# ishine/tts-max

Hardware: AMD Instinct MI355X
Metric: audio-codes/sec + RTF@24kHz, TTS-1 bs=1/32, at 1/2/4/8 MI355X (higher is better)
Workload: dtype bf16; 1 GPU; tts1 bf16 bs=1/GPU: prompt 202 tokens (150 codes), 500 greedy codes, codec codec-24k on 650 codes; model=TTS-1 (Llama-3.2-1B dims, V=193856, tied) + xcodec2-style codec codec-24k, global_batch=1, seq_len=702, parallelism=dp1

## Files before the change

### include/tts_mi355x_ops.h

```cpp
#ifndef TTS_MI355X_OPS_H
#define TTS_MI355X_OPS_H

#include <stdint.h>
#include "tts_mi355x.h"

#ifdef __cplusplus
extern "C" {
#endif

tts_status tts_synth_fill(void* dst, int32_t dtype, int64_t n, uint64_t seed, float scale,
                          void* stream);

tts_status tts_op_retile(const void* w, void* w_tiled, int32_t N, int32_t K, int32_t epi, void* stream);

tts_status tts_op_wgemm(const void* x, int32_t M, int32_t K, int32_t ldx, const void* w_tiled,
                        int32_t N, const void* normw, float eps, void* out, int32_t ldo,
                        void* resid, int32_t epi, void* stream);

tts_status tts_op_pgemm(const void* x, int32_t M, int32_t K, const void* w_tiled, int32_t N, void* out,
                        int32_t ldo, void* resid, int32_t epi, void* stream);

tts_status tts_op_head_pick(const void* x, int32_t M, int32_t K, const void* normw, float eps, const void* w_tiled,
                            int32_t N, const uint32_t* seen, int32_t seen_stride, float penalty,
                            const uint16_t* counts, float freq_penalty, const int32_t* eos_mask,
// ... 3 lines not shown
tts_status tts_op_sample(const float* logits, int32_t B, int32_t V, float temperature, int32_t top_k,
                         float top_p, uint64_t seed, int32_t step, const float* part_max, int32_t nparts,
                         float* probs, int32_t* tokens, void* stream);

tts_status tts_op_sample_list(const float* scores, const int32_t* ids, const int32_t* counts, int32_t B,
                              int32_t cap, int32_t V, float temperature, int32_t top_k, float top_p, uint64_t seed,
                              int32_t step, float* probs, int32_t* tokens, void* stream);

tts_status tts_op_sample_rows(const float* scores, const int32_t* ids, const int32_t* counts, int32_t B, int32_t cap,
                              int32_t V, const float* temperature, const int32_t* top_k, const float* top_p,
                              const int32_t* sample, const uint64_t* row_seed, int32_t step, const float* part_max,
                              const int32_t* part_idx, int32_t nparts, float* probs, int32_t* tokens, void* stream);

tts_status tts_debug_step_plan(const tts_lm_config* cfg, int32_t rows, int32_t num_cu, char* out, int32_t cap);
tts_status tts_debug_wgemm_plan(int32_t M, int32_t N, int32_t K, int32_t epi, int32_t num_cu, int32_t* out);
tts_status tts_debug_step_plan_sampled(const tts_lm_config* cfg, int32_t rows, int32_t num_cu, int32_t top_k,
                                       char* out, int32_t cap);

tts_status tts_debug_step_plan_rows(const tts_lm_config* cfg, int32_t rows, int32_t num_cu, int32_t max_top_k,
                                    char* out, int32_t cap);

tts_status tts_op_rmsnorm(const void* x, const void* w, float eps, void* y, int32_t M, int32_t K,
                          void* stream);

tts_status tts_op_attn_prefill(const void* qkv, int32_t ld_qkv, const int32_t* seq_slot, const int32_t* seq_pos0,
                               const int32_t* seq_len, int32_t n_seq, int32_t n_slots, void* kcache,
                               void* vtcache, int32_t max_seq, const void* rope_cos, const void* rope_sin,
                               int32_t H, int32_t KVH, int32_t D, float scale, void* q_rot, void* out,
                               void* stream);

// ... 15 lines not shown
```

### tts-max_amd/csrc/capi.cpp

```cpp
#include <stdlib.h>
#include <string.h>

#include <algorithm>
#include <memory>
#include <string>

#include "../../include/tts_mi355x.h"
#include "../../include/tts_mi355x_ops.h"
#include "codec_kernels.h"
#include "engine.h"

namespace tts {

static thread_local std::string g_last_error;

template <class F>
static tts_status guarded(F&& f) {
  try {
    f();
    return TTS_OK;
  } catch (const Error& e) {
    g_last_error = e.what();
    return e.code;
  } catch (const std::exception& e) {
// ... 242 lines not shown
}

tts_status tts_debug_wgemm_plan(int32_t M, int32_t N, int32_t K, int32_t epi, int32_t num_cu, int32_t* out) {
  return guarded([&] {
    TTS_REQUIRE(out && num_cu > 0, "null argument");
    TTS_REQUIRE(epi >= EPI_STORE && epi <= EPI_LOGITS_ROWS && wgemm_supported(M, N, K, epi), "unsupported GEMM shape");
    const WgemmPlan p = plan_wgemm(M, N, K, epi, num_cu);
    out[0] = (N / 16) / p.sp.ng;
    out[1] = p.sp.ur();
    out[2] = p.grid;
    out[3] = p.sp.kc;
    out[4] = p.csplit;
    out[5] = p.sliced ? 1 : 0;
    out[6] = p.a_lds ? 1 : 0;
    out[7] = p.cfg;
  });
}

tts_status tts_debug_step_plan_sampled(const tts_lm_config* cfg, int32_t rows, int32_t num_cu, int32_t top_k,
                                       char* out, int32_t cap) {
  return guarded([&] {
    TTS_REQUIRE(cfg && out && cap > 0, "null argument");
    TTS_REQUIRE(top_k >= 1 && top_k <= SAMPLE_MAX_TOP_K, "top_k in [1, 1024]");
    const std::string p = lm_step_plan(*cfg, rows, num_cu, top_k);
    TTS_REQUIRE((int64_t)p.size() < cap, "output buffer too small");
    memcpy(out, p.c_str(), p.size() + 1);
  });
}

tts_status tts_debug_step_plan_rows(const tts_lm_config* cfg, int32_t rows, int32_t num_cu, int32_t max_top_k,
// ... 415 lines not shown
```

### tts-max_amd/csrc/lm_debug.cpp

```cpp
#include "lm_step.h"

namespace tts {

#ifdef TTS_STAMPS
static unsigned long long* g_stamps = nullptr;
constexpr int kStampSlots = 1 << 16;
unsigned long long* stamp_buf() {
  if (!g_stamps) {
    HIP_CHECK(hipMalloc((void**)&g_stamps, kStampSlots * 8));
    HIP_CHECK(hipMemset(g_stamps, 0, kStampSlots * 8));
  }
  return g_stamps;
}
extern "C" int tts_debug_stamps(unsigned long long* host, int n) {
  if (!g_stamps || n > kStampSlots) return 1;
  if (hipDeviceSynchronize() != hipSuccess) return 1;
  if (hipMemcpy(host, g_stamps, (size_t)n * 8, hipMemcpyDeviceToHost) != hipSuccess) return 1;
  return hipMemset(g_stamps, 0, kStampSlots * 8) == hipSuccess ? 0 : 1;
}
#else
unsigned long long* stamp_buf() { return nullptr; }
#endif

void lm_bench_kernel(Engine* e, int which, int rows, int ctx, int iters, float* avg_ms,
                     double* bytes) {
  TTS_REQUIRE(e->lm.loaded, "tts_lm_load has not been called");
  TTS_REQUIRE(rows >= 1 && rows <= e->w.cap_batch, "rows out of range");
  TTS_REQUIRE(ctx >= 1 && ctx <= e->lm.cfg.max_seq_len, "ctx out of range");
  TTS_REQUIRE(which >= 0 && which <= 11 && iters >= 1, "bad kernel selector");
  hipStream_t s = e->stream;
  Ctx X(e, s);
  const tts_lm_config& c = X.c;
  const int HID = c.hidden_size, HD = c.num_heads * c.head_dim, FF = c.intermediate_size;
  const int V = c.vocab_size, QKV = X.QKV(), hgrid = X.M.head_grid;
  TTS_REQUIRE(which < 6 || which > 7 || X.fused_attn_ok(rows, true), "fused QKV+attention does not apply to this shape");
  TTS_REQUIRE(which != 10 || (hgrid && head_screen_topk_supported(rows, HID, V, 50, hgrid)),
              "the screened sampling head does not apply to this shape (or is off)");
  TTS_REQUIRE(which < 8 || which > 9 || (hgrid && rows <= 32 && head_screen_supported(rows, HID, V)),
              "the screened lm_head does not apply to this shape (or is off)");
  TTS_REQUIRE(which != 7 || (rows == 1 ? X.fused_oproj_ok() : X.fused_oproj_rows_ok(rows)),
              "fused o_proj does not apply to this shape (or is off)");
  std::vector<int> tok(rows), pos(rows, ctx - 1);
  for (int r = 0; r < rows; ++r) tok[r] = (r * 7919 + 11) % V;
  HIP_CHECK(hipMemcpyAsync(e->w.row_idx.p, tok.data(), rows * 4, hipMemcpyHostToDevice, s));
// ... 70 lines not shown
          X.pending_norm = nullptr;
          X.screened_sample(e->w.x.as<bf16_t>(), rows, st, sampled);
          b = (double)V * HID + 16.0 * V + act_rw * HID + rows * (V / 8.0);
        } else {
          X.pending_norm = nullptr;
          X.lm_head_pick(e->w.x.as<bf16_t>(), rows, sx, EPI_LOGITS, true);
          SampleArgs sa = X.sample_args(st, sampled, false, X.head_parts(rows, EPI_LOGITS, true));
          sa.out_part_val = nullptr; sa.out_part_idx = nullptr;
          sa.tokens = e->w.row_idx.as<int>();
          launch_sample(sa, rows, s);
          b = 2.0 * V * HID + act_rw * HID + 2.0 * HID + rows * (V / 8.0) + 2.0 * rows * V * 4.0;
        }
        launch_bump_epoch(st.epoch, s);
        break;
      }
    }
  };
  launch();
  HIP_CHECK(hipGetLastError());
  HIP_CHECK(hipEventRecord(e->ev[2], s));
  for (int i = 0; i < iters; ++i) launch();
  HIP_CHECK(hipEventRecord(e->ev[3], s));
  HIP_CHECK(hipEventSynchronize(e->ev[3]));
  float ms = 0.f;
  HIP_CHECK(hipEventElapsedTime(&ms, e->ev[2], e->ev[3]));
  *avg_ms = ms / iters;
  *bytes = b;
  read_device_flags(e, s);
}

// ... 87 lines not shown
```

### tts-max_amd/csrc/lm_gemm.hip

```cpp
#include <algorithm>
#include <cstdio>
#include <stdexcept>

#include "env.h"
#include "lm_gemm_kernel.h"

namespace tts {

std::vector<std::string>*& dry_launches() {
  static thread_local std::vector<std::string>* rec = nullptr;
  return rec;
}

__global__ void retile_kernel(const bf16_t* __restrict__ w, bf16_t* __restrict__ t, int N,
                              int K, int nt_mult, int nt_off, StreamPlan p, int units) {
  const int KT = K / 32;
  const long long nchunks = (long long)(N / 16) * KT * 64;
  const int ur = p.ur();
  for (long long c = blockIdx.x * (long long)blockDim.x + threadIdx.x; c < nchunks;
       c += (long long)gridDim.x * blockDim.x) {
    const int lane = (int)(c & 63);
    const long long tile = c >> 6;
    const int kt = (int)(tile % KT);
    const int nt = (int)(tile / KT);
// ... 127 lines not shown
  return M >= 1 && M <= 64 && N > 0 && K > 0 && (N % (16 * NG)) == 0 && (K % 256) == 0 &&
         (unsigned long long)N * (unsigned long long)K * 2ull <= kWgemmMaxBytes;
}

void launch_wgemm(const WgemmArgs& a_in, const WgemmPlan& p_in, int epi, bool norm, hipStream_t s) {
  WgemmArgs a = a_in;
  WgemmPlan p = p_in;
  if (p.csplit == 2 && a.fattn_wgs) {
    p.csplit = 1;
    p.grid = p.sp.grid;
  }
  a.ur = p.sp.ur();
  a.kc = p.sp.kc;
  a.sliced = p.sliced ? 1 : 0;
  a.csplit = p.csplit;
  if (a.csplit == 2 && epi != EPI_STORE && epi != EPI_RESID)
    throw std::runtime_error("wgemm: column split only for plain store / residual launches");
  static const int diag = env_int("TTS_WGEMM_DIAG", 0);
  a.diag = diag;
  if (p.sliced) {
    if (norm || (epi != EPI_STORE && epi != EPI_RESID) || (a.part_out == nullptr && !dry_launches()))
      throw std::runtime_error("K-sliced wgemm: store/residual epilogues with a partial workspace only");
    const int Kfull = a.K;
    a.K = Kfull / p.sp.kc;
    launch_wgemm_store(a, p, false, s);
    if (epi == EPI_RESID && a.next_norm && !a.norm_out && !dry_launches())
      throw std::runtime_error("K-sliced wgemm: next_norm without norm_out");
    if (epi == EPI_RESID && a.next_norm)
      launch_splitk_combine_norm(a.part_out, p.sp.kc, a.M, a.N, a.ldo, a.resid, a.ldo, a.next_norm, a.eps,
                                 a.norm_out, a.ldo, s);
// ... 17 lines not shown
```

### tts-max_amd/csrc/lm_gemm_kernel.h

```cpp
#pragma once
#include <algorithm>
#include <cstdio>
#include <stdexcept>
#include <type_traits>

#include "hip_common.h"
#include "lm_kernels.h"
#include "lm_attn_core.h"
#include "lm_logit_epilogue.h"

namespace tts {

constexpr int wgemm_ea(int waves) { return waves >= 16 ? 1 : (waves >= 8 ? 2 : 4); }
__host__ __device__ inline int wgemm_red_floats(int waves, int ksplit, int ng, int mt, int M, int Kl) {
  const int upw = waves / ksplit;
  int r = upw * (ksplit - 1) * ng * mt * 4 * 64;
  r = r > upw * mt * 16 * 2 ? r : upw * mt * 16 * 2;
  const int segs = (M * (Kl / 8) + 63) / 64;
  r = r > segs ? r : segs;
  r = r > Kl / 2 ? r : Kl / 2;
  return r + 64;
}

constexpr int wgemm_fattn_d(int ku) { return ku == 2 ? 64 : 128; }
// ... 215 lines not shown
      for (int j = 0; j < HB; ++j)
        if (p0 + j < KSPLIT) pv[j] = *(const f32x4_t*)(red + ((size_t)(p0 + j - 1) * 64 + lane) * 4);
#pragma unroll
      for (int j = 0; j < HB; ++j)
        if (p0 + j < KSPLIT) acc += pv[j];
    }
#pragma unroll
    for (int r = 0; r < 4; ++r) {
      const int m = 4 * (lane >> 4) + r;
      if (m < M) a.fo_resid[(size_t)m * hid + u * 16 + (lane & 15)] = f2bf(bf2f(rr[r]) + rbf(acc[r]));
    }
  }
  TTS_STAMP(stp, 3);
}


constexpr int A_GLOBAL = 0, A_LDS = 1;

template <int WAVES, int KU, int MT_MAX, int NG, int KSPLIT, int ASRC, bool NORM, int EPI, int R,
          bool EARLY, int KSW = KSPLIT, bool FROWS = false>
__global__ __launch_bounds__(WAVES * 64) void wgemm_kernel(WgemmArgs a) {
  extern __shared__ __attribute__((aligned(16))) char smem[];
  constexpr int NT = WAVES * 64;
  constexpr bool LOGITS = EPI == EPI_LOGITS || EPI == EPI_LOGITS_ROWS;
  constexpr bool FATT = EPI == EPI_STORE && ASRC == A_LDS && WAVES == DEC_NW && KSW == KSPLIT && MT_MAX == 1 &&
                        ((EARLY && !FROWS && wgemm_fattn_d(KU) == 64) || (!EARLY && FROWS));
#ifdef TTS_STAMPS
  const unsigned long long t_first = __builtin_amdgcn_s_memrealtime();
#endif
  asm volatile("" ::"s"(a.x), "s"(a.w), "s"(a.normw), "s"(a.resid), "s"(a.stamps), "s"(a.M), "s"(a.K), "s"(a.ldx),
               "s"(a.N), "s"(a.ldo), "s"(a.ur));
  asm volatile("" ::"s"(a.fattn_wgs), "s"(a.fo_units), "s"(a.csplit), "s"(a.sliced), "s"(a.diag), "s"(a.KT), "s"(a.Sc),
               "s"(a.S), "s"(a.units), "s"(a.nproj), "s"(a.ur_div.mul), "s"(a.ur_div.shift), "s"(a.kch_div.mul),
               "s"(a.kch_div.shift), "s"(a.sc_div.mul), "s"(a.sc_div.shift));
  const int nproj = FROWS ? (int)gridDim.x - a.fattn_wgs - (a.fattn_wgs ? a.fo_units : 0) : a.nproj;
  if constexpr (FATT) {
    const int cb = (int)blockIdx.x - nproj;
    if (FROWS ? a.fattn_wgs != 0 : cb >= 0) {
      if (cb >= 0 && cb < a.fattn_wgs) {
        fattn_consumer<NT, wgemm_fattn_d(KU)>(a, smem, cb);
        return;
      }
      if (cb >= a.fattn_wgs) {
        const int lane = threadIdx.x & 63;
        const int wave = __builtin_amdgcn_readfirstlane(threadIdx.x >> 6);
        const size_t xs_bytes = (((size_t)a.M * (a.K + 8) * 2 + 15) & ~(size_t)15);
        if constexpr (FROWS) {
          fused_oproj_rows<KU, KSPLIT, R>(a, (bf16_t*)smem, (float*)(smem + xs_bytes), wave, lane, cb - a.fattn_wgs);
        } else {
          const uint32_t tag = ((uint32_t)a.fa.row_pos[0] << 6) | (uint32_t)a.fattn_layer;
          fused_oproj<KU, KSPLIT, R>(a, (bf16_t*)smem, (float*)(smem + xs_bytes), wave, lane, tag, cb - a.fattn_wgs);
        }
        return;
      }
    }
  }
// ... 23 lines not shown
  const int st_off = SL > 1 ? 0 : by * Sc;
  const int kt_base = by * (a.K >> 5);
  const bf16_t* xg = a.x + (uint32_t)(by * a.K);
  const int ldxs = a.K + 8;
  const int ustride = nproj * UPW;

  bf16_t* xs = (bf16_t*)smem;
  const size_t xs_bytes = (ASRC != A_GLOBAL) ? (((size_t)M * ldxs * 2 + 15) & ~(size_t)15) : 0;
  float* red = (float*)(smem + xs_bytes);

  const int ur = a.ur;
  auto stile = [&](int uu, int st) -> long long {
    uu = min(uu, units - 1) >> cs2;
    const int r = (int)fastdiv((uint32_t)uu, a.ur_div), ui = uu - r * ur;
    const int nr = min(ur, bunits - r * ur);
    return (long long)r * ur * KT * NG + (((long long)(st + st_off) * nr + ui) * KSPLIT + kpart) * NG * KU;
  };
  const int S = a.S;

  const int tid = threadIdx.x;
  const int kch = a.K >> 3;
  constexpr bool FTAGS = FATT && !EARLY;
  int ftag_pos = 0;
  if constexpr (FTAGS) {
    if (a.fattn_wgs) ftag_pos = a.fa.row_pos[min(lane & 15, M - 1)];
  }
  constexpr int EA = wgemm_ea(WAVES);
  const int achunks = M * kch;
  const int a_nj = (achunks + NT - 1) / NT;
  constexpr bool early_a = EARLY && ASRC == A_LDS;
  u32x4_t xe[EA], ne[EA];
// ... 495 lines not shown
      throw std::runtime_error("wgemm: fused one-row attention: head dim 64 only");
    if (a.fo_units && a.M > 1) {
      const int HD = a.fa.H * a.fa.D;
      const int S = (HD / 32) / (KSPLIT * KU);
      if (!(a.fo_w && a.fo_resid && a.fo_units <= a.fo_ur && S == R && KSPLIT == WAVES && HD == a.K && a.fo_kc >= 1 &&
            (HD / 32) % (a.fo_kc * KSPLIT * KU) == 0 && R * KU % 4 == 0 && R * KU >= 4))
        throw std::runtime_error("wgemm: fused multi-row o_proj shape mismatch");
    } else if (a.fo_units) {
      const int S = (a.fa.H * a.fa.D / 32) / (KSPLIT * KU);
      if (!(a.fo_w && a.fo_resid && a.fo_units <= a.fo_ur && S == R && a.fa.H * a.fa.D == KSPLIT * 128 &&
            KSPLIT == WAVES && (size_t)a.M * (a.K + 8) * 2 >= (size_t)KSPLIT * 256))
        throw std::runtime_error("wgemm: fused o_proj shape mismatch");
    }
    lds = std::max(lds, a.fa.D == 64 ? fattn_lds_bytes<64>() : fattn_lds_bytes<128>());
    grid += a.fattn_wgs + a.fo_units;
  }
  if (lds > 160 * 1024) throw std::runtime_error("wgemm: LDS request above 160 KiB");
  if ((unsigned long long)a.N * (unsigned long long)(a.sliced ? (size_t)a.K * a.kc : (size_t)a.K) * 2ull > kWgemmMaxBytes)
    throw std::runtime_error("wgemm: tiled weight matrix above the 32-bit buffer range");
  if (ASRC == A_LDS && !EARLY && a.K % 512 != 0)
    throw std::runtime_error("wgemm: the LDS-DMA prologue needs K a multiple of 512 (plan_wgemm: A_GLOBAL)");
  wgemm_derive(a, KU, NG, KSPLIT, KSPLIT, nproj, ASRC != A_GLOBAL);
  const dim3 g(grid, a.sliced ? a.kc : 1);
  if (!a.x) throw std::runtime_error("wgemm: launch without an A operand");
  if (g.y != 1 && !a.sliced) throw std::runtime_error("wgemm: grid.y > 1 on an unsliced launch");
  if (frows) {
    if constexpr (EPI == EPI_STORE && ASRC == A_LDS && WAVES == DEC_NW)
      hipLaunchKernelGGL((wgemm_kernel<WAVES, KU, 1, NG, KSPLIT, ASRC, NORM, EPI, R, false, KSPLIT, true>), g,
                         dim3(WAVES * 64), lds, s, a);
  } else if (mt == 1)
// ... 13 lines not shown
  if (a.M <= 16 && !(a.fattn_wgs && a.M > 1)) {
    const int kch = a.K / 8, NT = WAVES * 64;
    if (ASRC == A_LDS) early = (kch % 64 == 0) && (a.M * kch + NT - 1) / NT <= wgemm_ea(WAVES);
  }
  if constexpr (ASRC == A_GLOBAL) launch_one_e<WAVES, KU, NG, KSPLIT, ASRC, NORM, EPI, R, false>(a, grid, s);
  else if (early) launch_one_e<WAVES, KU, NG, KSPLIT, ASRC, NORM, EPI, R, true>(a, grid, s);
  else launch_one_e<WAVES, KU, NG, KSPLIT, ASRC, NORM, EPI, R, false>(a, grid, s);
}

template <int C, int NG, int ASRC, bool NORM, int EPI>
static void launch_shape(const WgemmArgs& a, int grid, hipStream_t s) {
  constexpr Shape3 h = kShapes[C];
  const int S = (a.K / 32) / (h.ksplit * h.ku);
  const bool agr_r1 = ASRC == A_GLOBAL && (h.ku >= 4 || (a.M > 16 && h.ku > 2));
  if constexpr (NG == 2 && ASRC == A_LDS && h.ku == 2 && h.waves == 8) {
    if (a.M >= 4 && a.M <= 32 && S % 4 == 0) {
      launch_one<h.waves, h.ku, NG, h.ksplit, ASRC, NORM, EPI, 4>(a, grid, s);
      return;
    }
  }
  if (h.r >= 2 && S % 2 == 0 && !agr_r1) launch_one<h.waves, h.ku, NG, h.ksplit, ASRC, NORM, EPI, 2>(a, grid, s);
  else launch_one<h.waves, h.ku, NG, h.ksplit, ASRC, NORM, EPI, 1>(a, grid, s);
}

template <int NG, int ASRC, bool NORM, int EPI>
static void launch_cfg(const WgemmArgs& a, int cfg, int grid, hipStream_t s) {
  if constexpr (NG == 2) {
    switch (cfg) {
      case 4: launch_shape<4, NG, ASRC, NORM, EPI>(a, grid, s); break;
      case 6: launch_shape<6, NG, ASRC, NORM, EPI>(a, grid, s); break;
      default: launch_shape<5, NG, ASRC, NORM, EPI>(a, grid, s); break;
// ... 19 lines not shown
```

### tts-max_amd/csrc/lm_gemm_swiglu.hip

```cpp
#include "lm_gemm_kernel.h"

namespace tts {

void launch_wgemm_swiglu(const WgemmArgs& a, const WgemmPlan& p, bool norm, hipStream_t s) {
  if (!p.a_lds) launch_cfg<2, A_GLOBAL, false, EPI_SWIGLU>(a, p.cfg, p.grid, s);
  else if (norm) launch_cfg<2, A_LDS, true, EPI_SWIGLU>(a, p.cfg, p.grid, s);
  else launch_cfg<2, A_LDS, false, EPI_SWIGLU>(a, p.cfg, p.grid, s);
}

}
```

### tts-max_amd/csrc/lm_kernels.h

```cpp
#pragma once
#include <hip/hip_runtime.h>
#include <stddef.h>
#include <stdint.h>

#include <stdexcept>
#include <string>
#include <vector>

#include "fastdiv.h"

namespace tts {

std::vector<std::string>*& dry_launches();
inline bool dry_record(const std::string& what) {
  std::vector<std::string>* v = dry_launches();
  if (!v) return false;
  v->push_back(what);
  return true;
}

typedef uint16_t bf16_t;

enum { EPI_STORE = 0, EPI_RESID = 1, EPI_SWIGLU = 2, EPI_LOGITS = 3, EPI_LOGITS_ROWS = 4 };

// ... 6 lines not shown
struct StreamPlan {
  int ng = 1, ksplit = 1, ku = 8, waves = 4, grid = 1, kc = 1;
  __host__ __device__ int ur() const { return grid * (waves / ksplit); }
};
__host__ __device__ inline long long plan_tile(int ng, int ksplit, int ku, int ur, int units, int KT,
                                               int kc, int nt, int kt) {
  const int u = nt / ng, g = nt - u * ng;
  const int KTc = KT / kc, kt_pc = KTc / ksplit;
  const int c = kt / KTc, rr = kt - c * KTc;
  const int kp = rr / kt_pc, ki = rr - kp * kt_pc;
  const int st = c * (kt_pc / ku) + ki / ku, kk = ki % ku;
  const int r = u / ur, ui = u - r * ur;
  const int nr = (units - r * ur) < ur ? (units - r * ur) : ur;
  return (long long)r * ur * KT * ng +
         (((long long)st * nr * ksplit + (long long)ui * ksplit + kp) * ng + g) * ku + kk;
}
StreamPlan stream_plan(int N, int K, int ng, int num_cu);
constexpr int LOGITS_MAX_PARTS = 1024;

struct AttnArgs {
  const bf16_t* qkv = nullptr;
  int ld_qkv = 0;
  int rows = 0;
  const int* row_slot = nullptr;
  const int* row_pos = nullptr;
  bf16_t* kcache = nullptr;
  bf16_t* vtcache = nullptr;
  int max_seq = 0;
  const bf16_t* rope_cos = nullptr;
  const bf16_t* rope_sin = nullptr;
// ... 18 lines not shown
  uint32_t* seen;
  int seen_stride;
  int* out_ids;
  int out_stride;
  int* n_active;
  uint16_t* counts;
  unsigned long long* row_seed;
  uint32_t* epoch;
  int eos_id;
  int min_new;
  const RowParams* par = nullptr;
};

constexpr unsigned long long kWgemmMaxBytes = 0xFFFF0000ull;
constexpr uint32_t kWgemmSentinel = 0xFFFFFFF0u;

struct alignas(64) WgemmArgs {
  const bf16_t* x = nullptr;
  const bf16_t* w = nullptr;
  const bf16_t* normw = nullptr;
  bf16_t* resid = nullptr;
  unsigned long long* stamps = nullptr;
  int M = 0, K = 0, ldx = 0;
  int N = 0;
  int ldo = 0;
  int ur = 0;
  int fattn_wgs = 0;
  int fo_units = 0;
  int csplit = 1;
  int sliced = 0;
// ... 23 lines not shown
  const RowParams* row_par = nullptr;
  float* part_out = nullptr;
  const bf16_t* next_norm = nullptr;
  bf16_t* norm_out = nullptr;
  uint64_t* gran = nullptr;
  AttnArgs fa;
  FastDiv kvh_div;
  int fattn_layer = 0;
  int* fattn_err = nullptr;
  int fattn_spins = 1 << 16;
  const bf16_t* fo_w = nullptr;
  int fo_ur = 0, fo_kc = 1;
  int fo_Sc = 0;
  FastDiv fo_sc_div;
  bf16_t* fo_resid = nullptr;
};
static_assert(offsetof(WgemmArgs, eps) == 128, "WgemmArgs: the prologue's fields fill the first two 64-byte lines");
static_assert(offsetof(WgemmArgs, x) == 0 && offsetof(WgemmArgs, w) == 8, "WgemmArgs: x, w lead (tests/test_wgemm_prologue_isa.py)");
static_assert(offsetof(WgemmArgs, fattn_wgs) == 64, "WgemmArgs: line 1 starts at the role split");

inline void wgemm_derive(WgemmArgs& a, int ku, int ng, int ksplit, int ksw, int nproj, bool a_lds) {
  const int sl = ksplit / ksw;
  const int kc = a.kc;
  a.KT = a.sliced ? (a.K >> 5) * kc : (a.K >> 5) * sl;
  const int KTc = a.KT / kc, kt_pc = KTc / ksplit;
  a.Sc = kt_pc / ku;
  if (a.ur < 1 || a.Sc < 1 || a.Sc * ku * ksplit * kc != a.KT)
    throw std::runtime_error("wgemm: K does not divide into the plan's stages");
  if (a.csplit != 1 && a.csplit != 2) throw std::runtime_error("wgemm: csplit is 1 or 2");
  a.S = a.sliced ? a.Sc : kc * a.Sc;
// ... 13 lines not shown
      a.fo_Sc = ((HD >> 5) / a.fo_kc) / ksplit / ku;
      const int fo_S = (HD >> 5) / (ksplit * ku);
      ok = a.fo_Sc > 0 && fastdiv_make((uint32_t)a.fo_Sc, (uint32_t)fo_S, &a.fo_sc_div) && ok;
    }
  }
  if (!ok) throw std::runtime_error("wgemm: no exact multiply-high pair for a launch divisor");
}

struct WgemmPlan {
  StreamPlan sp;
  int cfg = 0;
  int grid = 1;
  bool a_lds = true;
  bool sliced = false;
  int csplit = 1;
};

void launch_retile(const bf16_t* w, bf16_t* t, int N, int K, int N_total, int ng, int num_cu,
                   hipStream_t s, int nt_mult = 1, int nt_off = 0);
WgemmPlan plan_wgemm(int M, int N, int K, int epi, int num_cu);
size_t wgemm_lds_bytes(int waves, int ksplit, int ng, int M, int Kl, bool a_in_lds);
inline size_t wgemm_part_elems(const WgemmPlan& p, int M, int ldo) {
  return p.sliced ? (size_t)p.sp.kc * M * ldo : 0;
}
bool wgemm_supported(int M, int N, int K, int epi);
bool wgemm_fattn_ok(int N, int K, int num_cu);
bool wgemm_fattn_rows_ok(int M, int N, int K, int D, int num_cu);
void launch_wgemm(const WgemmArgs& a, const WgemmPlan& p, int epi, bool norm, hipStream_t s);
void launch_wgemm_kslice(const WgemmArgs& a, int units, hipStream_t s);

struct HeadScreenArgs {
// ... 161 lines not shown
```

### tts-max_amd/csrc/lm_step.cpp

```cpp
#include "lm_step.h"

namespace tts {

static bool head_screen_wait(int rows, bool sampled = false) {
  static const int v = env_int("TTS_HEAD_SCREEN_WAIT", -1);
  if (v < 0) return sampled || rows >= 2;
  return v == 1 || (v > 1 && rows >= v);
}
bool head_screen_check() { static const bool v = env_set("TTS_HEAD_SCREEN_CHECK"); return v; }

static bool use_fused_attn() { static const bool v = env_on("TTS_FUSED_ATTN"); return v; }
static bool use_fused_oproj() { static const bool v = env_on("TTS_FUSED_OPROJ"); return v; }

static bool use_qkv_defer() { static const bool v = env_on("TTS_QKV_DEFER"); return v; }
static bool use_kslice32() { static const bool v = env_on("TTS_KSLICE32"); return v; }
static bool use_fused_oproj_rows() { static const bool v = env_on("TTS_FUSED_OPROJ_ROWS"); return v; }

static bool use_wide_head() { static const bool v = env_on("TTS_WIDE_HEAD"); return v; }

StepState step_state_row(const StepState& st, int slot) {
  StepState one = st;
  one.tokens += slot; one.pos += slot; one.gen_count += slot; one.limit += slot;
  one.done += slot; one.eos_mask += slot; one.row_seed += slot;
  if (one.par) one.par += slot;
// ... 43 lines not shown
    a.part = w.ppart.as<float>(); a.part_bytes = w.ppart.bytes;
    if (resid == w.x.as<bf16_t>() && ldo == c.hidden_size && next_norm) {
      a.next_norm = next_norm; a.eps = c.rms_norm_eps; a.xn = w.xn.as<bf16_t>();
    }
    if (launch_pgemm(a, epi, e->num_cu, s)) pending_norm = next_norm;
    return false;
  }
  const int chunk = rows > 32 ? 32 : kPrefillChunk;
  for (int r0 = 0; r0 < rows; r0 += chunk) {
    const int m = std::min(chunk, rows - r0);
    WgemmPlan p = plan_wgemm(m, N, K, epi, e->num_cu);
    if (p.sliced && wgemm_part_elems(p, m, ldo) * 4 > w.kpart.bytes) {
      p.sliced = false;
      p.a_lds = false;
    }
    const bf16_t* xin = x ? x + (size_t)r0 * K : nullptr;
    bool norm = normw != nullptr;
    if (norm && normw == ready && x == w.x.as<bf16_t>()) {
      xin = w.xn.as<bf16_t>() + (size_t)r0 * K;
      norm = false;
    } else if (norm && (!p.a_lds || p.sliced || K > 4096 || rows > 16)) {
      launch_rmsnorm(xin, K, normw, c.rms_norm_eps, w.xn.as<bf16_t>(), K, m, K, s);
      xin = w.xn.as<bf16_t>();
      norm = false;
    }
    if (!norm && rows > 16 && m <= 32 && K == 2048 && !logit_extra &&
        (epi == EPI_STORE || epi == EPI_RESID) && use_kslice32() && p.sp.kc == 1 && p.sp.waves == 16 && p.sp.ksplit == 16 && p.sp.ku == 2 && p.sp.ng == 1 &&
        (size_t)4 * m * ldo * 4 <= w.kpart.bytes) {
      WgemmArgs a;
      a.x = xin; a.M = m; a.K = K / 4; a.ldx = K;
// ... 64 lines not shown
  a.blocks = w.blocks.as<int4>(); a.nblocks = w.nblocks;
  a.stamps = stamp_buf();
  if (qkv_part) {
    a.qkv_part = w.kpart.as<float>();
    a.qkv_nsl = 4;
  }
  return a;
}

bool Ctx::fused_attn_ok(int rows, bool decode) const {
  if (!decode || !use_fused_attn() || c.num_layers < 2 || c.num_layers > 64) return false;
  if (rows == 1) return c.head_dim == 64 && wgemm_fattn_ok(QKV(), c.hidden_size, e->num_cu);
  static const int max_rows = env_int("TTS_FATTN_ROWS", 16);
  return rows <= std::min(16, max_rows) && wgemm_fattn_rows_ok(rows, QKV(), c.hidden_size, c.head_dim, e->num_cu);
}
WgemmArgs Ctx::fused_attn_args(const AttnArgs& a, int layer, bool with_oproj) {
  WgemmArgs fx;
  fx.gran = w.gran.as<uint64_t>();
  fx.fa = a;
  fx.fattn_wgs = a.rows * a.KVH;
  fx.fattn_layer = layer;
  fx.fattn_err = w.ferr.as<int>() + FERR_GRANULE_TIMEOUT;
  static const int spins = std::max(1, env_int("TTS_FATTN_SPINS", 1 << 16));
  fx.fattn_spins = spins;
  if (with_oproj) {
    const LmLayer& ly = M.layers[layer];
    const WgemmPlan po = plan_wgemm(a.rows, c.hidden_size, c.num_heads * c.head_dim, EPI_RESID, e->num_cu);
    fx.fo_w = ly.wo;
    fx.fo_units = c.hidden_size / 16;
    fx.fo_ur = po.sp.ur();
    fx.fo_kc = po.sp.kc;
    fx.fo_resid = w.x.as<bf16_t>();
  }
  return fx;
}
bool Ctx::fused_oproj_ok() const {
  if (!use_fused_oproj()) return false;
  const int HD = c.num_heads * c.head_dim, HID = c.hidden_size;
  const WgemmPlan pq = plan_wgemm(1, QKV(), HID, EPI_STORE, e->num_cu);
  const WgemmPlan po = plan_wgemm(1, HID, HD, EPI_RESID, e->num_cu);
  const StreamPlan& s = po.sp;
  return s.waves == 16 && s.ku == 2 && s.ksplit == 16 && s.kc == 1 && s.ng == 1 && HD == 16 * 128 &&
         (HD / 32) / (s.ksplit * s.ku) == 2 && HID / 16 <= s.ur() && HID / 16 <= pq.sp.grid &&
         pq.sp.waves == 16 && pq.sp.ku == 2 && pq.sp.ksplit == 16;
}

bool Ctx::fused_oproj_rows_ok(int rows) const {
// ... 284 lines not shown
```

### tts-max_amd/csrc/lm_step.h

```cpp
#pragma once
#include <math.h>
#include <string.h>

#include <algorithm>
#include <cstdio>

#include "engine.h"

namespace tts {

constexpr int kPrefillChunk = 64;
constexpr int kMaxPrefillRows = 8192;

size_t kpart_bytes(const tts_lm_config& c);
size_t ppart_bytes(const tts_lm_config& c);
int head_screen_grid(const tts_lm_config& c, int num_cu);
bool head_screen_check();
unsigned long long* stamp_buf();
void read_device_flags(Engine* e, hipStream_t s);

enum { ST_TOKENS, ST_POS, ST_GEN_COUNT, ST_LIMIT, ST_DONE, ST_EOS_MASK, ST_N_ACTIVE };
inline int st_at(int array, int B, int b) { return array * B + b; }
inline std::vector<int> st_zeros(int B) { return std::vector<int>(st_at(ST_N_ACTIVE, B, B) + 1, 0); }
StepState step_state_row(const StepState& st, int slot);
// ... 36 lines not shown
  }
  void lm_head_pick(const bf16_t* x, int rows, const WgemmArgs& epilogue, int epi = EPI_LOGITS, bool tile_head = false) {
    Gemm g{x, rows, c.hidden_size, M.lm_head, c.vocab_size, epi};
    g.normw = M.final_norm; g.extra = &epilogue; g.tile_head = tile_head;
    gemm(g);
  }
  void lm_head_logits(const bf16_t* x, int rows, bf16_t* out) {
    Gemm g{x, rows, c.hidden_size, M.lm_head, c.vocab_size, EPI_STORE};
    g.out = out; g.ldo = c.vocab_size; g.normw = M.final_norm;
    gemm(g);
  }

  AttnArgs attn_args(int layer, int rows, const int* slot, const int* pos, bool qkv_part = false);
  bool fused_attn_ok(int rows, bool decode) const;
  WgemmArgs fused_attn_args(const AttnArgs& a, int layer, bool with_oproj = false);
  bool fused_oproj_ok() const;
  bool fused_oproj_rows_ok(int rows) const;
  void layers(int rows, const int* slot, const int* pos, bool decode);

  StepState state(int B, int eos, int min_new);
  WgemmArgs head_epilogue_args(const StepState& st, const tts_gen_params& gp);
  SampleArgs sample_args(const StepState& st, const tts_gen_params& gp, bool lists, int nparts = 0);
  void head_and_pick(const bf16_t* xin, int B, const StepState& st, const tts_gen_params& gp, bool step = false);
  int head_parts(int B, int epi, bool step) const;
  bool rows_screen_ok(int B, int max_top_k) const;
  void head_and_pick_rows(const bf16_t* xin, int B, const StepState& st, bool dense, int max_top_k);
  void screened_sample(const bf16_t* xin, int B, const StepState& st, const tts_gen_params& gp);
  int screened_head_parts(const bf16_t* xin, int B, const StepState& st, const tts_gen_params& gp, int top_k = 0,
                          const RowParams* par = nullptr);

// ... 34 lines not shown
```

### tts-max_amd/tts_amd/_lib.py

```python

from __future__ import annotations

import ctypes
import os

import torch

_HERE = os.path.dirname(os.path.abspath(__file__))
LIB_PATH = os.environ.get("TTS_LIB_PATH") or os.path.join(_HERE, "libtts_mi355x.so")

TTS_OK = 0
TTS_E_INVALID = 1
TTS_E_STATE = 4
DT_F32, DT_BF16, DT_F16, DT_I32, DT_I64 = 0, 1, 2, 3, 4
EPI_STORE, EPI_RESID, EPI_SWIGLU = 0, 1, 2

EXPORTED_SYMBOLS = (
    "tts_abi_version",
    "tts_last_error",
    "tts_engine_create",
    "tts_engine_destroy",
    "tts_lm_load",
    "tts_generate",
    "tts_generate_begin",
# ... 10 lines not shown
    "tts_lm_id_to_code",
    "tts_lm_last_timing",
    "tts_lm_bench_kernel",
    "tts_codec_load",
    "tts_codec_decode",
    "tts_codec_samples_per_code",
    "tts_encoder_load",
    "tts_encoder_encode",
    "tts_encoder_encode_features",
    "tts_synth_fill",
    "tts_op_retile",
    "tts_op_wgemm",
    "tts_debug_step_plan",
    "tts_debug_wgemm_plan",
    "tts_debug_step_plan_sampled",
    "tts_op_pgemm",
    "tts_op_sample",
    "tts_op_sample_list",
    "tts_op_sample_rows",
    "tts_slots_open_per_request",
    "tts_slots_add_params",
    "tts_debug_step_plan_rows",
    "tts_op_rmsnorm",
    "tts_op_gemm_f32",
    "tts_op_attn_prefill",
    "tts_op_attn_decode",
    "tts_op_head_pick",
)


# ... 119 lines not shown
        "tts_op_retile": (I32, [P, P, I32, I32, I32, P]),
        "tts_op_wgemm": (I32, [P, I32, I32, I32, P, I32, P, F32, P, I32, P, I32, P]),
        "tts_op_pgemm": (I32, [P, I32, I32, P, I32, P, I32, P, I32, P]),
        "tts_op_head_pick": (I32, [P, I32, I32, P, F32, P, I32, P, I32, F32, P, F32, P, P, P, P, P, pi32, P, I32, P]),
        "tts_op_sample": (I32, [P, I32, I32, F32, I32, F32, ctypes.c_uint64, I32, P, I32, P, P, P]),
        "tts_op_sample_list": (I32, [P, P, P, I32, I32, I32, F32, I32, F32, ctypes.c_uint64, I32, P, P, P]),
        "tts_op_sample_rows": (I32, [P, P, P, I32, I32, I32, P, P, P, P, P, I32, P, P, I32, P, P, P]),
        "tts_op_rmsnorm": (I32, [P, P, F32, P, I32, I32, P]),
        "tts_op_gemm_f32": (I32, [P, I32, I32, I32, P, I32, P, P, I32, P, I32, P]),
        "tts_op_attn_prefill": (I32, [P, I32, pi32, pi32, pi32, I32, I32, P, P, I32, P, P, I32, I32, I32, F32, P, P, P]),
        "tts_op_attn_decode": (I32, [P, P, I32, I32, I32, P, P, I32, P, P, I32, P, P, I32, I32, I32, F32, P, P]),
        "tts_debug_step_plan": (I32, [ctypes.POINTER(LmConfig), I32, I32, ctypes.c_char_p, I32]),
        "tts_debug_wgemm_plan": (I32, [I32, I32, I32, I32, I32, pi32]),
        "tts_debug_step_plan_sampled": (I32, [ctypes.POINTER(LmConfig), I32, I32, I32, ctypes.c_char_p, I32]),
        "tts_debug_step_plan_rows": (I32, [ctypes.POINTER(LmConfig), I32, I32, I32, ctypes.c_char_p, I32]),
    }
    for name, (res, args) in sig.items():
        if os.environ.get("TTS_LIB_PATH") and not hasattr(lib, name):
            continue
        fn = getattr(lib, name)
        fn.restype = res
        fn.argtypes = args
    _lib = lib
    return lib


def check(status: int) -> None:
    if status != TTS_OK:
        msg = load_library().tts_last_error().decode(errors="replace")
        raise TtsError(status, msg)
# ... 30 lines not shown
```

### tts-max_amd/tts_amd/speechlm.py

```python

from __future__ import annotations

import ctypes
import dataclasses
import json
import math
import os
import threading
from typing import Any, Sequence

import numpy as np
import torch

from . import _lib, configs, synth


def hf_rope_table(arch: configs.LmArch, max_seq_len: int) -> tuple[torch.Tensor, torch.Tensor]:
    dim = arch.head_dim
    inv_freq = 1.0 / (arch.rope_theta ** (torch.arange(0, dim, 2, dtype=torch.int64).to(dtype=torch.float) / dim))
    if arch.rope_llama3:
        factor, lo, hi = arch.rope_factor, arch.rope_low_freq_factor, arch.rope_high_freq_factor
        old = arch.rope_original_max_position
        low_freq_wavelen = old / lo
        high_freq_wavelen = old / hi
# ... 287 lines not shown
            _lib.check(self._lib.tts_lm_score_decode(self._h, flat.ctypes.data_as(pi32), lens.ctypes.data_as(pi32), B,
                                                     n_last, gptr, k,
                                                     out.ctypes.data_as(ctypes.POINTER(ctypes.c_float)), None))
            return torch.from_numpy(out)

    def last_timing(self) -> tuple[float, float, int]:
        a, b, n = ctypes.c_float(), ctypes.c_float(), ctypes.c_int32()
        _lib.check(self._lib.tts_lm_last_timing(self._h, ctypes.byref(a), ctypes.byref(b), ctypes.byref(n)))
        return a.value, b.value, n.value

    KERNELS = ("qkv", "o_proj", "gate_up", "down", "lm_head", "attention")

    def bench_kernel(self, which: str, rows: int = 1, ctx: int = 450, iters: int = 50) -> tuple[float, float]:
        ms, b = ctypes.c_float(), ctypes.c_double()
        sel = {"qkv_attn": 6, "qkv_attn_oproj": 7, "head_screened": 8, "head_screen": 9,
               "sample_screened": 10, "sample_full": 11}.get(which)
        sel = self.KERNELS.index(which) if sel is None else sel
        _lib.check(self._lib.tts_lm_bench_kernel(self._h, sel, rows, ctx, iters,
                                                 ctypes.byref(ms), ctypes.byref(b)))
        return ms.value, b.value

    def ids_to_codes(self, ids: Sequence[int]) -> list[int]:
        arr = np.ascontiguousarray(np.asarray(ids, dtype=np.int32))
        out = np.zeros_like(arr)
        pi32 = ctypes.POINTER(ctypes.c_int32)
        _lib.check(self._lib.tts_lm_id_to_code(self._h, arr.ctypes.data_as(pi32), len(arr), out.ctypes.data_as(pi32)))
        return out.tolist()

    def close(self):
        if getattr(self, "_h", None):
            self._lib.tts_engine_destroy(self._h)
# ... 24 lines not shown
```

Before: 1801 audio-codes/s.

## Prefetch gate_up weights into L2 from warm workgroups in fused attention launch

Adds extra warm-up workgroups to the one-row fused QKV+attention+o_proj launch. They stream the first stages of the next gate_up weight matrix into cache with buffer-load-to-LDS, spread across XCDs, so the following gate_up GEMM starts from warm L2. It also enables a 4-deep ring variant of the gate_up kernel for the single-row case. The warm workgroups use CU time and bandwidth during attention and could contend with it. Debug entry points and a bench selector are added as well.

```diff
diff --git a/include/tts_mi355x_ops.h b/include/tts_mi355x_ops.h
--- a/include/tts_mi355x_ops.h
+++ b/include/tts_mi355x_ops.h
@@ -41,6 +41,8 @@
 
 tts_status tts_debug_step_plan(const tts_lm_config* cfg, int32_t rows, int32_t num_cu, char* out, int32_t cap);
 tts_status tts_debug_wgemm_plan(int32_t M, int32_t N, int32_t K, int32_t epi, int32_t num_cu, int32_t* out);
+tts_status tts_debug_warm_plan(int32_t N, int32_t K, int32_t num_cu, int32_t stages, int32_t wgs, int32_t shift,
+                               int32_t* info, int64_t* out, int32_t cap, int32_t* n);
 tts_status tts_debug_step_plan_sampled(const tts_lm_config* cfg, int32_t rows, int32_t num_cu, int32_t top_k,
                                        char* out, int32_t cap);
 
diff --git a/tts-max_amd/csrc/capi.cpp b/tts-max_amd/csrc/capi.cpp
--- a/tts-max_amd/csrc/capi.cpp
+++ b/tts-max_amd/csrc/capi.cpp
@@ -280,6 +280,27 @@
     out[5] = p.sliced ? 1 : 0;
     out[6] = p.a_lds ? 1 : 0;
     out[7] = p.cfg;
+  });
+}
+
+tts_status tts_debug_warm_plan(int32_t N, int32_t K, int32_t num_cu, int32_t stages, int32_t wgs, int32_t shift,
+                               int32_t* info, int64_t* out, int32_t cap, int32_t* n) {
+  return guarded([&] {
+    TTS_REQUIRE(info && out && n && num_cu > 0 && cap >= 0, "null argument");
+    TTS_REQUIRE(wgemm_supported(1, N, K, EPI_SWIGLU), "unsupported GEMM shape");
+    const WgemmPlan p = plan_wgemm(1, N, K, EPI_SWIGLU, num_cu);
+    const WarmArgs a = wgemm_warm_plan(p, nullptr, N, K, stages, wgs, shift);
+    const int32_t v[8] = {a.stages, a.wgs, a.nblk, (int32_t)a.blk_bytes, (int32_t)a.last_bytes, (int32_t)a.stage_bytes,
+                          a.shift, (K / 32) / (p.sp.ksplit * p.sp.ku)};
+    memcpy(info, v, sizeof v);
+    int rows = 0;
+    for (int b = 0; b < a.wgs; ++b)
+      warm_walk(a, b, [&](uint32_t off, uint32_t len, int g, int st) {
+        TTS_REQUIRE(rows < cap, "output buffer too small");
+        int64_t* r = out + (size_t)rows++ * 5;
+        r[0] = b; r[1] = off; r[2] = len; r[3] = g; r[4] = st;
+      });
+    *n = rows;
   });
 }
 
diff --git a/tts-max_amd/csrc/lm_debug.cpp b/tts-max_amd/csrc/lm_debug.cpp
--- a/tts-max_amd/csrc/lm_debug.cpp
+++ b/tts-max_amd/csrc/lm_debug.cpp
@@ -27,7 +27,7 @@
   TTS_REQUIRE(e->lm.loaded, "tts_lm_load has not been called");
   TTS_REQUIRE(rows >= 1 && rows <= e->w.cap_batch, "rows out of range");
   TTS_REQUIRE(ctx >= 1 && ctx <= e->lm.cfg.max_seq_len, "ctx out of range");
-  TTS_REQUIRE(which >= 0 && which <= 11 && iters >= 1, "bad kernel selector");
+  TTS_REQUIRE(which >= 0 && which <= 12 && iters >= 1, "bad kernel selector");
   hipStream_t s = e->stream;
   Ctx X(e, s);
   const tts_lm_config& c = X.c;
@@ -128,6 +128,11 @@
         launch_bump_epoch(st.epoch, s);
         break;
       }
+      case 12:
+        launch_warm_probe(X.warm_args(ly.wgu, 0), s);
+        X.gate_up(rows, ly);
+        b = 2.0 * 2 * FF * HID + act_rw * (HID + FF) + 2.0 * HID;
+        break;
     }
   };
   launch();
diff --git a/tts-max_amd/csrc/lm_gemm.hip b/tts-max_amd/csrc/lm_gemm.hip
--- a/tts-max_amd/csrc/lm_gemm.hip
+++ b/tts-max_amd/csrc/lm_gemm.hip
@@ -165,6 +165,7 @@
   a.kc = p.sp.kc;
   a.sliced = p.sliced ? 1 : 0;
   a.csplit = p.csplit;
+  a.ring = p.ring;
   if (a.csplit == 2 && epi != EPI_STORE && epi != EPI_RESID)
     throw std::runtime_error("wgemm: column split only for plain store / residual launches");
   static const int diag = env_int("TTS_WGEMM_DIAG", 0);
diff --git a/tts-max_amd/csrc/lm_gemm_kernel.h b/tts-max_amd/csrc/lm_gemm_kernel.h
--- a/tts-max_amd/csrc/lm_gemm_kernel.h
+++ b/tts-max_amd/csrc/lm_gemm_kernel.h
@@ -253,6 +253,36 @@
   TTS_STAMP(stp, 3);
 }
 
+TTS_DEV void warm_role(const WgemmArgs& a, char* smem, int b) {
+  unsigned long long* stp = a.stamps ? a.stamps + (size_t)blockIdx.x * 32 : nullptr;
+  TTS_STAMP(stp, 0);
+  const WarmArgs& wm = a.warm;
+  const uint32_t lane16 = (threadIdx.x & 63) * 16u;
+  const uint32_t wave = (uint32_t)__builtin_amdgcn_readfirstlane(threadIdx.x >> 6);
+  const uint32_t nwav = blockDim.x >> 6;
+  const __amdgpu_buffer_rsrc_t rs = __builtin_amdgcn_make_buffer_rsrc((void*)wm.w, (short)0, (int)wm.bytes, 0x00020000);
+  warm_walk(wm, b, [&](uint32_t off, uint32_t len, int, int) {
+    for (uint32_t q = wave * 1024u; q < len; q += nwav * 1024u)
+      __builtin_amdgcn_raw_ptr_buffer_load_lds(rs, (lptr_t)smem, 16, (int)lane16, (int)(off + q), 0, 0);
+  });
+  TTS_STAMP(stp, 1);
+  asm volatile("s_waitcnt vmcnt(0)" ::: "memory");
+  TTS_STAMP(stp, 3);
+}
+
+#ifdef TTS_STAMPS
+constexpr int kXccHist = 49152, kXccBlocks = 512, kXccLast = kXccHist - 1, kXccDist = kXccHist + 2 * kXccBlocks * 8;
+TTS_DEV void xcc_record(unsigned long long* stamps, int kind) {
+  if (!stamps || threadIdx.x != 0 || blockIdx.x >= kXccBlocks || blockIdx.y != 0) return;
+  const unsigned xcc = __builtin_amdgcn_s_getreg((3 << 11) | 20) & 7u;
+  atomicAdd(stamps + kXccHist + ((size_t)kind * kXccBlocks + blockIdx.x) * 8 + xcc, 1ull);
+  if (blockIdx.x == 0) {
+    if (kind == 0) stamps[kXccLast] = xcc + 1;
+    else if (stamps[kXccLast]) atomicAdd(stamps + kXccDist + ((xcc + 8 - (unsigned)(stamps[kXccLast] - 1)) & 7u), 1ull);
+  }
+}
+#endif
+
 
 constexpr int A_GLOBAL = 0, A_LDS = 1;
 
@@ -266,6 +296,11 @@
                         ((EARLY && !FROWS && wgemm_fattn_d(KU) == 64) || (!EARLY && FROWS));
 #ifdef TTS_STAMPS
   const unsigned long long t_first = __builtin_amdgcn_s_memrealtime();
+  if constexpr (FATT && EARLY && !FROWS) {
+    if (a.fattn_wgs) xcc_record(a.stamps, 0);
+  } else if constexpr (EPI == EPI_SWIGLU && MT_MAX == 1) {
+    if (a.M == 1) xcc_record(a.stamps, 1);
+  }
 #endif
   asm volatile("" ::"s"(a.x), "s"(a.w), "s"(a.normw), "s"(a.resid), "s"(a.stamps), "s"(a.M), "s"(a.K), "s"(a.ldx),
                "s"(a.N), "s"(a.ldo), "s"(a.ur));
@@ -279,6 +314,12 @@
       if (cb >= 0 && cb < a.fattn_wgs) {
         fattn_consumer<NT, wgemm_fattn_d(KU)>(a, smem, cb);
         return;
+      }
+      if constexpr (!FROWS) {
+        if (cb >= a.fattn_wgs + a.fo_units) {
+          warm_role(a, smem, cb - a.fattn_wgs - a.fo_units);
+          return;
+        }
       }
       if (cb >= a.fattn_wgs) {
         const int lane = threadIdx.x & 63;
@@ -332,7 +373,7 @@
     uu = min(uu, units - 1) >> cs2;
     const int r = (int)fastdiv((uint32_t)uu, a.ur_div), ui = uu - r * ur;
     const int nr = min(ur, bunits - r * ur);
-    return (long long)r * ur * KT * NG + (((long long)(st + st_off) * nr + ui) * KSPLIT + kpart) * NG * KU;
+    return wgemm_stage_tile(r, ui, nr, st + st_off, kpart, ur, KT, NG, KSPLIT, KU);
   };
   const int S = a.S;
 
@@ -858,6 +899,11 @@
     }
     lds = std::max(lds, a.fa.D == 64 ? fattn_lds_bytes<64>() : fattn_lds_bytes<128>());
     grid += a.fattn_wgs + a.fo_units;
+    if (a.warm.wgs && !(EARLY && a.M == 1 && a.fo_units && a.warm.w && a.warm.stages > 0 && a.warm.nblk > 0))
+      throw std::runtime_error("wgemm: warm workgroups ride the one-row launch that carries o_proj");
+    grid += a.warm.wgs;
+  } else if (a.warm.wgs) {
+    throw std::runtime_error("wgemm: warm workgroups without the fused launch");
   }
   if (lds > 160 * 1024) throw std::runtime_error("wgemm: LDS request above 160 KiB");
   if ((unsigned long long)a.N * (unsigned long long)(a.sliced ? (size_t)a.K * a.kc : (size_t)a.K) * 2ull > kWgemmMaxBytes)
@@ -901,7 +947,7 @@
   const int S = (a.K / 32) / (h.ksplit * h.ku);
   const bool agr_r1 = ASRC == A_GLOBAL && (h.ku >= 4 || (a.M > 16 && h.ku > 2));
   if constexpr (NG == 2 && ASRC == A_LDS && h.ku == 2 && h.waves == 8) {
-    if (a.M >= 4 && a.M <= 32 && S % 4 == 0) {
+    if (((a.M >= 4 && a.M <= 32) || (a.M == 1 && a.ring == 4)) && S % 4 == 0) {
       launch_one<h.waves, h.ku, NG, h.ksplit, ASRC, NORM, EPI, 4>(a, grid, s);
       return;
     }
diff --git a/tts-max_amd/csrc/lm_gemm_swiglu.hip b/tts-max_amd/csrc/lm_gemm_swiglu.hip
--- a/tts-max_amd/csrc/lm_gemm_swiglu.hip
+++ b/tts-max_amd/csrc/lm_gemm_swiglu.hip
@@ -8,4 +8,16 @@
   else launch_cfg<2, A_LDS, false, EPI_SWIGLU>(a, p.cfg, p.grid, s);
 }
 
+__global__ __launch_bounds__(DEC_NW * 64) void warm_probe_kernel(WgemmArgs a) {
+  extern __shared__ __attribute__((aligned(16))) char smem[];
+  warm_role(a, smem, (int)blockIdx.x);
 }
+void launch_warm_probe(const WarmArgs& warm, hipStream_t s) {
+  if (warm.wgs <= 0) return;
+  if (!warm.w || warm.stages <= 0 || warm.nblk <= 0) throw std::runtime_error("warm probe: empty plan");
+  WgemmArgs a;
+  a.warm = warm;
+  hipLaunchKernelGGL(warm_probe_kernel, dim3(warm.wgs), dim3(DEC_NW * 64), 1024, s, a);
+}
+
+}
diff --git a/tts-max_amd/csrc/lm_kernels.h b/tts-max_amd/csrc/lm_kernels.h
--- a/tts-max_amd/csrc/lm_kernels.h
+++ b/tts-max_amd/csrc/lm_kernels.h
@@ -44,6 +44,10 @@
   const int nr = (units - r * ur) < ur ? (units - r * ur) : ur;
   return (long long)r * ur * KT * ng +
          (((long long)st * nr * ksplit + (long long)ui * ksplit + kp) * ng + g) * ku + kk;
+}
+__host__ __device__ inline long long wgemm_stage_tile(int r, int ui, int nr, int st, int kpart, int ur, int KT,
+                                                      int ng, int ksplit, int ku) {
+  return (long long)r * ur * KT * ng + (((long long)st * nr + ui) * ksplit + kpart) * ng * ku;
 }
 StreamPlan stream_plan(int N, int K, int ng, int num_cu);
 constexpr int LOGITS_MAX_PARTS = 1024;
@@ -92,6 +96,33 @@
 
 constexpr unsigned long long kWgemmMaxBytes = 0xFFFF0000ull;
 constexpr uint32_t kWgemmSentinel = 0xFFFFFFF0u;
+
+struct WarmArgs {
+  const bf16_t* w = nullptr;
+  uint32_t bytes = 0;
+  int wgs = 0;
+  int stages = 0;
+  int nblk = 0;
+  uint32_t blk_bytes = 0, last_bytes = 0, stage_bytes = 0;
+  int shift = 0;
+};
+constexpr int kWarmXcds = 8;
+constexpr uint32_t kWarmMaxBytesPerXcd = 3u << 20;
+template <typename F>
+__host__ __device__ inline void warm_walk(const WarmArgs& a, int b, F f) {
+  const int c = (b + a.shift) & (kWarmXcds - 1);
+  const int nw = (a.wgs - (b & (kWarmXcds - 1)) + kWarmXcds - 1) / kWarmXcds;
+  const int nb = c < a.nblk ? (a.nblk - c + kWarmXcds - 1) / kWarmXcds : 0;
+  if (nb == 0 || nw <= 0) return;
+  int st = 0, i = b / kWarmXcds;
+  for (;;) {
+    while (i >= nb && st < a.stages) { i -= nb; ++st; }
+    if (st >= a.stages) return;
+    const int g = c + kWarmXcds * i;
+    f((uint32_t)st * a.stage_bytes + (uint32_t)g * a.blk_bytes, g == a.nblk - 1 ? a.last_bytes : a.blk_bytes, g, st);
+    i += nw;
+  }
+}
 
 struct alignas(64) WgemmArgs {
   const bf16_t* x = nullptr;
@@ -145,6 +176,8 @@
   int fo_Sc = 0;
   FastDiv fo_sc_div;
   bf16_t* fo_resid = nullptr;
+  int ring = 0;
+  WarmArgs warm;
 };
 static_assert(offsetof(WgemmArgs, eps) == 128, "WgemmArgs: the prologue's fields fill the first two 64-byte lines");
 static_assert(offsetof(WgemmArgs, x) == 0 && offsetof(WgemmArgs, w) == 8, "WgemmArgs: x, w lead (tests/test_wgemm_prologue_isa.py)");
@@ -188,7 +221,39 @@
   bool a_lds = true;
   bool sliced = false;
   int csplit = 1;
-};
+  int ring = 0;
+};
+
+inline WarmArgs wgemm_warm_plan(const WgemmPlan& p, const bf16_t* w, int N, int K, int W, int wgs, int shift) {
+  const StreamPlan& s = p.sp;
+  if (wgs < 0 || (wgs > 0 && wgs < kWarmXcds)) throw std::runtime_error("warm plan: 0 or at least 8 warm workgroups");
+  if (p.sliced || p.csplit != 1 || p.grid != s.grid || N <= 0 || K <= 0 || N % (16 * s.ng) || K % (32 * s.ksplit * s.ku) ||
+      (unsigned long long)N * (unsigned long long)K * 2ull > kWgemmMaxBytes)
+    throw std::runtime_error("warm plan: not a plain one-round-order launch of a tiled matrix");
+  const int upw = s.waves / s.ksplit, units = (N / 16) / s.ng, KT = K / 32, ur = s.ur();
+  const int S = KT / (s.ksplit * s.ku);
+  const int nr = ur < units ? ur : units;
+  auto at = [&](int ui, int st) {
+    return (uint32_t)((unsigned long long)wgemm_stage_tile(0, ui, nr, st, 0, ur, KT, s.ng, s.ksplit, s.ku) * 1024ull);
+  };
+  WarmArgs a;
+  a.w = w;
+  a.bytes = (uint32_t)((unsigned long long)(N / 16) * KT * 1024ull);
+  a.nblk = (nr + upw - 1) / upw;
+  a.blk_bytes = at(upw, 0);
+  a.last_bytes = at(nr - (a.nblk - 1) * upw, 0);
+  a.stage_bytes = at(0, 1);
+  const uint32_t per_xcd = (uint32_t)((a.nblk + kWarmXcds - 1) / kWarmXcds) * a.blk_bytes;
+  const int fit = (int)(kWarmMaxBytesPerXcd / per_xcd);
+  W = W < S ? W : S;
+  W = W < fit ? W : fit;
+  a.stages = (wgs > 0 && W > 0) ? W : 0;
+  a.wgs = a.stages ? wgs : 0;
+  a.shift = ((shift % kWarmXcds) + kWarmXcds) % kWarmXcds;
+  return a;
+}
+
+void launch_warm_probe(const WarmArgs& warm, hipStream_t s);
 
 void launch_retile(const bf16_t* w, bf16_t* t, int N, int K, int N_total, int ng, int num_cu,
                    hipStream_t s, int nt_mult = 1, int nt_off = 0);
diff --git a/tts-max_amd/csrc/lm_step.cpp b/tts-max_amd/csrc/lm_step.cpp
--- a/tts-max_amd/csrc/lm_step.cpp
+++ b/tts-max_amd/csrc/lm_step.cpp
@@ -81,6 +81,7 @@
       p.sliced = false;
       p.a_lds = false;
     }
+    if (epi == EPI_SWIGLU && rows == 1 && gate_up_ring4()) p.ring = 4;
     const bf16_t* xin = x ? x + (size_t)r0 * K : nullptr;
     bool norm = normw != nullptr;
     if (norm && normw == ready && x == w.x.as<bf16_t>()) {
@@ -175,6 +176,18 @@
   static const int max_rows = env_int("TTS_FATTN_ROWS", 16);
   return rows <= std::min(16, max_rows) && wgemm_fattn_rows_ok(rows, QKV(), c.hidden_size, c.head_dim, e->num_cu);
 }
+bool Ctx::gate_up_ring4() const {
+  static const bool on = env_int("TTS_GU_RING", 4) != 2;
+  return on && fused_attn_ok(1, true) && fused_oproj_ok();
+}
+WarmArgs Ctx::warm_args(const bf16_t* wgu, int first_block) const {
+  static const int stages = env_int("TTS_WARM_STAGES", 2);
+  static const int wgs = env_int("TTS_WARM_WGS", 120);
+  static const int dist = env_int("TTS_WARM_XCD_DIST", 0);
+  if (stages <= 0 || wgs < kWarmXcds) return WarmArgs{};
+  const WgemmPlan pg = plan_wgemm(1, 2 * c.intermediate_size, c.hidden_size, EPI_SWIGLU, e->num_cu);
+  return wgemm_warm_plan(pg, wgu, 2 * c.intermediate_size, c.hidden_size, stages, wgs, first_block - dist);
+}
 WgemmArgs Ctx::fused_attn_args(const AttnArgs& a, int layer, bool with_oproj) {
   WgemmArgs fx;
   fx.gran = w.gran.as<uint64_t>();
@@ -192,6 +205,8 @@
     fx.fo_ur = po.sp.ur();
     fx.fo_kc = po.sp.kc;
     fx.fo_resid = w.x.as<bf16_t>();
+    if (a.rows == 1)
+      fx.warm = warm_args(ly.wgu, plan_wgemm(1, QKV(), c.hidden_size, EPI_STORE, e->num_cu).sp.grid + fx.fattn_wgs + fx.fo_units);
   }
   return fx;
 }
diff --git a/tts-max_amd/csrc/lm_step.h b/tts-max_amd/csrc/lm_step.h
--- a/tts-max_amd/csrc/lm_step.h
+++ b/tts-max_amd/csrc/lm_step.h
@@ -74,6 +74,8 @@
   AttnArgs attn_args(int layer, int rows, const int* slot, const int* pos, bool qkv_part = false);
   bool fused_attn_ok(int rows, bool decode) const;
   WgemmArgs fused_attn_args(const AttnArgs& a, int layer, bool with_oproj = false);
+  WarmArgs warm_args(const bf16_t* wgu, int first_block) const;
+  bool gate_up_ring4() const;
   bool fused_oproj_ok() const;
   bool fused_oproj_rows_ok(int rows) const;
   void layers(int rows, const int* slot, const int* pos, bool decode);
diff --git a/tts-max_amd/tts_amd/_lib.py b/tts-max_amd/tts_amd/_lib.py
--- a/tts-max_amd/tts_amd/_lib.py
+++ b/tts-max_amd/tts_amd/_lib.py
@@ -48,6 +48,7 @@
     "tts_debug_step_plan",
     "tts_debug_wgemm_plan",
     "tts_debug_step_plan_sampled",
+    "tts_debug_warm_plan",
     "tts_op_pgemm",
     "tts_op_sample",
     "tts_op_sample_list",
@@ -197,6 +198,7 @@
         "tts_debug_wgemm_plan": (I32, [I32, I32, I32, I32, I32, pi32]),
         "tts_debug_step_plan_sampled": (I32, [ctypes.POINTER(LmConfig), I32, I32, I32, ctypes.c_char_p, I32]),
         "tts_debug_step_plan_rows": (I32, [ctypes.POINTER(LmConfig), I32, I32, I32, ctypes.c_char_p, I32]),
+        "tts_debug_warm_plan": (I32, [I32, I32, I32, I32, I32, I32, pi32, ctypes.POINTER(ctypes.c_int64), I32, pi32]),
     }
     for name, (res, args) in sig.items():
         if os.environ.get("TTS_LIB_PATH") and not hasattr(lib, name):
diff --git a/tts-max_amd/tts_amd/speechlm.py b/tts-max_amd/tts_amd/speechlm.py
--- a/tts-max_amd/tts_amd/speechlm.py
+++ b/tts-max_amd/tts_amd/speechlm.py
@@ -325,7 +325,7 @@
     def bench_kernel(self, which: str, rows: int = 1, ctx: int = 450, iters: int = 50) -> tuple[float, float]:
         ms, b = ctypes.c_float(), ctypes.c_double()
         sel = {"qkv_attn": 6, "qkv_attn_oproj": 7, "head_screened": 8, "head_screen": 9,
-               "sample_screened": 10, "sample_full": 11}.get(which)
+               "sample_screened": 10, "sample_full": 11, "warm_gate_up": 12}.get(which)
         sel = self.KERNELS.index(which) if sel is None else sel
         _lib.check(self._lib.tts_lm_bench_kernel(self._h, sel, rows, ctx, iters,
                                                  ctypes.byref(ms), ctypes.byref(b)))
```

Result: faster. 1861 audio-codes/s, median of 6 (+3.3%).
